# Black-Phoenix/CUDA-SfM

Hardware: AMD Instinct MI355X
Metric: RANSAC E-matrix hypotheses/sec (8-point, fused scoring), inlier-mask parity vs CPU oracle (higher is better)
Workload: dtype f32

## Files before the change

### cuda-sfm_amd/csrc/common.hpp

```cpp
#pragma once
#include <hip/hip_runtime.h>
#include <stdint.h>
#include <stddef.h>
#include <string>
#include <atomic>
#include <type_traits>
#include "../../include/sfm_amd.h"
#include "pair_state.hpp"
#include "job_order.hpp"
#if SFM_AB
#include "../../include/sfm_amd_ab.h"
#endif

#if SFM_AB
#define SFM_SW(p, i) ((p).reserved[i])
#else
#define SFM_SW(p, i) 0
#endif

namespace sfm {

void set_error(const char *fmt, ...);

#define SFM_HIP_TRY(expr)                                                                      \
// ... 143 lines not shown
    size_t views_floats = 0;
    hipEvent_t views_ev = nullptr;
    float pool_K[9] = {}, pool_Kinv[9] = {};
    float *pool_records = nullptr;
    size_t pool_records_cap = 0;
    void *batch_ws = nullptr;
    size_t batch_ws_bytes = 0;
    sfm::JobArray refine_jobs, register_jobs, view_points_jobs, adjust_jobs, align_jobs, fuse_jobs, chain_jobs, ring_jobs;
    void *fuse_ws = nullptr;
    size_t fuse_ws_bytes = 0;
    void *chain_ws = nullptr;
    size_t chain_ws_bytes = 0;
    void *ring_ws = nullptr;
    size_t ring_ws_bytes = 0;
    void *sift_job = nullptr;
    static constexpr int kBigLdsSlots = 16;
    const void *big_lds_done[kBigLdsSlots] = {};
};

inline int allow_big_lds(sfm_ctx *ctx, const void *kernel)
{
    for (int i = 0; i < sfm_ctx::kBigLdsSlots; ++i) {
        if (ctx->big_lds_done[i] == kernel) return SFM_OK;
        if (ctx->big_lds_done[i] == nullptr) {
            SFM_HIP_TRY(hipFuncSetAttribute(kernel, hipFuncAttributeMaxDynamicSharedMemorySize, 160 * 1024));
            ctx->big_lds_done[i] = kernel;
            return SFM_OK;
        }
    }
    SFM_HIP_TRY(hipFuncSetAttribute(kernel, hipFuncAttributeMaxDynamicSharedMemorySize, 160 * 1024));
    return SFM_OK;
}

struct ShardSlot {
    int *counts = nullptr;
    uint32_t *tick = nullptr;
    float *Ecand = nullptr;
    void *pf = nullptr;
    unsigned long long *key = nullptr;
    size_t cap_hyps = 0;
};

inline void shard_slot_free(ShardSlot &s)
{
    for (void *b : { (void *)s.counts, (void *)s.tick, (void *)s.Ecand, s.pf, (void *)s.key }) if (b) (void)hipFree(b);
    s = ShardSlot();
}

struct sfm_pair {
    sfm_ctx *ctx = nullptr;
    int image_count = 2;
    int n = 0;
    int cap_points = 0;
    int ld = 0;
    float *d_K = nullptr, *d_Kinv = nullptr;
    float *d_U[2] = { nullptr, nullptr };
    float *d_X[2] = { nullptr, nullptr };
    float4 *d_pts4 = nullptr;
    uint32_t sorted_epoch = 0;
    uint32_t pf_seen_epoch = 0;
    int pf_rule = 0;
    uint32_t *d_buckets = nullptr;
    size_t bucket_words = 0;
    uint32_t *d_tile_boxes = nullptr;
    int boxes_words = 0, boxes_tile = 0;
    float4 *d_pts4s = nullptr;
// ... 32 lines not shown
    float *d_vstate = nullptr;
    float *d_vreproj = nullptr;
    void *d_vwork = nullptr;
    void *d_vhyp = nullptr;
    int *d_vcounts = nullptr;
    size_t cap_vhyps = 0;
    uint32_t view_hyps = 0;
    void *d_awork = nullptr;
    void *d_lwork = nullptr;
    void *d_lhyp = nullptr;
    size_t cap_lhyps = 0;
    int last_kernel = 0, last_grid = 0, last_block = 0, last_lds = 0;
};

namespace sfm {

int match_db_rows(const sfm_ctx *ctx, int n2);
int match_records(sfm_ctx *ctx, sfm_sift_point *d_sift1, int n1, const sfm_sift_point *d_sift2, int n2, int *out_idx);
int pose_chain(sfm_pair *pair, int mode, float *d_record);

int lane_contexts(sfm_ctx *ctx, int n, sfm_ctx **out);
int start_lanes_after(sfm_ctx *ctx, sfm_ctx *const *lanes, int n, hipEvent_t event);

int launch_ransac_score(sfm_pair *pair, ShardSlot &slot, hipStream_t stream, const sfm_ransac_params &p, uint32_t h0, uint32_t count,
                        unsigned long long *key2 = nullptr, const float *d_E_given = nullptr, bool serial = true);
int launch_ransac_finalize(sfm_pair *pair, const sfm_ransac_params &p, const unsigned long long *d_key, uint32_t hyp_host, bool from_key,
                           hipStream_t stream = nullptr, bool rederive = false);
int launch_permutation_indices(sfm_ctx *ctx, int n, uint32_t seed, int32_t *d_indices);
bool prefilter_usable(const sfm_pair *pair, const sfm_ransac_params &p, uint32_t count);
int prefilter_pick_rule(sfm_pair *pair, const sfm_ransac_params &p, uint32_t count);
int launch_score_prefilter(sfm_pair *pair, ShardSlot &slot, hipStream_t stream, const sfm_ransac_params &p, uint32_t h0, uint32_t count, unsigned long long *key2);
bool prefilter_sums_counts(const sfm_pair *pair, const sfm_ransac_params &p, uint32_t count);
int launch_pf_prep(sfm_pair *pair, ShardSlot &slot, hipStream_t stream, const sfm_ransac_params &p, uint32_t count);
int prefilter_tile_points(const sfm_pair *pair, const sfm_ransac_params &p);
int launch_pf_cells(sfm_pair *pair, hipStream_t stream, bool want_sorted = false, int tile = 0);
#if SFM_AB
int launch_score_prefilter_r2(sfm_pair *pair, ShardSlot &slot, hipStream_t stream, const sfm_ransac_params &p, uint32_t h0, uint32_t count, unsigned long long *key2);
int launch_score_mfma(sfm_pair *pair, ShardSlot &slot, hipStream_t stream, const sfm_ransac_params &p, uint32_t h0, uint32_t count);
int launch_prefilter_probe(sfm_ctx *ctx, const float *d_E, float thr, float B, const float pt[4], int survive_all, float *d_out);
int launch_prefilter_band_probe(sfm_ctx *ctx, const float *d_E, float thr, float B, const float box[8], int b_safe, const float pt[4], int survive_all, float *d_out);
#endif
int launch_ransac_fused(sfm_pair *pair, ShardSlot &slot, hipStream_t stream, const sfm_ransac_params &p, uint32_t h0, uint32_t count);
int launch_finalize_block(sfm_pair *pair, const sfm_ransac_params &p, const unsigned long long *d_key, uint32_t hyp_host, bool from_key,
                          hipStream_t stream, bool rederive);

int launch_fill_xu(sfm_pair *pair, const sfm_sift_point *d_data);
int launch_set_points(sfm_pair *pair, const float *d_X0, const float *d_X1);
int launch_pose_candidates(sfm_pair *pair, int mode);
int launch_choose_pose(sfm_pair *pair, int mode);
int launch_triangulate(sfm_pair *pair, int mode);
int launch_points_to_vbo(sfm_pair *pair, float *d_positions, float *d_velocities, float scale);
int launch_pair_record(sfm_pair *pair, int mode, float *d_record);
int launch_pose_chain(sfm_pair *pair, float *d_record);

int launch_refine(sfm_pair *pair, const sfm_refine_params &p);
int launch_refine_pairs(sfm_ctx *ctx, sfm_pair *const *pairs, int num_pairs, const sfm_refine_params &p, const uint8_t *const *d_masks);
size_t refine_work_bytes(int cap_points);
int refine_state_words();
int refine_pose_offset();
int refine_report_offset();

int launch_register(sfm_pair *pair, const sfm_sift_point *d_sift, const sfm_register_params &p, const float *d_points, const uint8_t *d_valid);
int launch_register_views(sfm_ctx *ctx, sfm_pair *const *pairs, int num_pairs, const sfm_sift_point *const *d_sifts, const sfm_register_params &p,
                          const float *const *d_points, const uint8_t *const *d_valid);
size_t register_work_bytes(int cap_points);
size_t register_hyp_bytes(size_t num_hypotheses);
// ... 75 lines not shown
```

### cuda-sfm_amd/csrc/prefilter_lds.hpp

```cpp
#pragma once
#include "prefilter_record.hpp"

namespace sfm {

constexpr int kPfTileMax = 1024;
constexpr int kPfWaves = 16;
constexpr int kPfRing = 128;

constexpr int kPfERow = 10;
constexpr int kPfPassRows = 32, kPfPairRows = 64;
constexpr int pf_wave_bytes(int rows) { return rows * kPfERow * 4 + rows * 4; }
template <int RULE> struct PfLds {
    static constexpr int kFragsPerBlock = RULE == kPfRuleG ? 3 : 2;
    static constexpr int kBlockBytes = kFragsPerBlock * 64 * 16;
    static constexpr int kFrag = 0;
    static constexpr int kTileMax = kPfTileMax;
    int staged, pts, ring, wave, next, lut, bytes;
    __host__ __device__ explicit PfLds(int tile, int ring_entries = kPfRing, int entry_bytes = 8, int rows = RULE == kPfRuleG ? kPfPassRows : kPfPairRows)
    {
        staged = (tile + 63) & ~63;
        pts = kFrag + (staged / 32) * kBlockBytes;
        ring = pts + staged * 16;
        ring = (ring + ring_entries * entry_bytes - 1) & ~(ring_entries * entry_bytes - 1);
        wave = ring + kPfWaves * ring_entries * entry_bytes;
        next = wave + kPfWaves * pf_wave_bytes(rows);
        lut = next + 16;
        bytes = lut + kPfRingLutBytes;
    }
};
static_assert(kPfRing * 8 == 1024, "ring slots are addressed with (offset & 1023) | base");

static inline int pf_tile_points(int ld, int tmax)
{
    const int ntiles = (ld + tmax - 1) / tmax;
    const int t = ((ld + ntiles - 1) / ntiles + 31) & ~31;
    return t < 32 ? 32 : t;
}

constexpr unsigned long long kPfSumCountsMin = 1ull << 21;
static inline bool pf_sums_counts_at(unsigned count, int ld, int tile)
{
    return (unsigned long long)count * (unsigned long long)((ld + tile - 1) / tile) >= kPfSumCountsMin;
}

constexpr unsigned long long kPfPairPassesMin = 1ull << 22;
static inline bool pf_pairs_passes_at(unsigned count, int ld, int tile)
{
    return (unsigned long long)count * (unsigned long long)((ld + tile - 1) / tile) >= kPfPairPassesMin;
}

}
```

### cuda-sfm_amd/csrc/ransac.hip

```cpp
#include "ransac_device.hpp"
#include "block_ops.hpp"
#include "prefilter_record.hpp"

namespace sfm {

__device__ __forceinline__ void reset_keys(unsigned long long *key, unsigned long long *key2)
{
    if (blockIdx.x == 0 && threadIdx.x == 0) {
        key[0] = 0ull; key[1] = 0ull;
        if (key2) *key2 = 0ull;
    }
}

template <int WPE>
__global__ __launch_bounds__(64, WPE)
void ransac_solve_lanes(const float *__restrict__ X0, const float *__restrict__ X1, int ld, int n,
                        const int32_t *__restrict__ indices, uint32_t seed, uint32_t h0, uint32_t count,
                        int sweeps, float *__restrict__ Ecand, unsigned long long *zero_key, unsigned long long *zero_key2,
                        int *__restrict__ zero_counts, uint32_t *__restrict__ zero_ticks, uint32_t nzero)
{
    reset_keys(zero_key, zero_key2);
    const uint32_t i = blockIdx.x * blockDim.x + threadIdx.x;
    if (zero_ticks) for (uint32_t w = i; w < nzero; w += gridDim.x * blockDim.x) zero_ticks[w] = 0u;
    if (i >= count) return;
// ... 209 lines not shown
        unsigned long long b = sbest[0];
#pragma unroll
        for (int w = 1; w < WPB; ++w) b = sbest[w] > b ? sbest[w] : b;
        if (b) {
            atomicMax(best_key, b);
            if (best_key2) atomicMax(best_key2, b);
        }
    }
}

__global__ __launch_bounds__(256)
void ransac_argmax_counts(const int *__restrict__ counts, uint32_t h0, uint32_t count,
                          unsigned long long *best_key, unsigned long long *best_key2)
{
    __shared__ unsigned long long sbest[4];
    unsigned long long b = 0;
    for (uint32_t i = blockIdx.x * blockDim.x + threadIdx.x; i < count; i += gridDim.x * blockDim.x) {
        const unsigned long long key = pack_key((uint32_t)counts[i], h0 + i);
        b = key > b ? key : b;
    }
    b = wave_max(b);
    if ((threadIdx.x & 63) == 0) sbest[threadIdx.x >> 6] = b;
    __syncthreads();
    if (threadIdx.x == 0) {
#pragma unroll
        for (int w = 1; w < 4; ++w) b = sbest[w] > b ? sbest[w] : b;
        if (b) {
            atomicMax(best_key, b);
            if (best_key2) atomicMax(best_key2, b);
        }
    }
}

static size_t tick_words(size_t count) { return 2 * count + 64; }

static int ensure_hyp_capacity(ShardSlot &s, hipStream_t stream, size_t count)
{
    if (count <= s.cap_hyps) return SFM_OK;
    SFM_HIP_TRY(hipStreamSynchronize(stream));
    for (void *b : { (void *)s.counts, (void *)s.Ecand, (void *)s.tick, s.pf }) if (b) (void)hipFree(b);
    s.counts = nullptr; s.Ecand = nullptr; s.tick = nullptr; s.pf = nullptr; s.cap_hyps = 0;
    SFM_HIP_TRY(hipMalloc(&s.tick, tick_words(count) * sizeof(uint32_t)));
    SFM_HIP_TRY(hipMalloc(&s.pf, count * sizeof(PfRecord)));
    SFM_HIP_TRY(hipMalloc(&s.counts, count * sizeof(int)));
    SFM_HIP_TRY(hipMalloc(&s.Ecand, count * 9 * sizeof(float)));
    s.cap_hyps = count;
    return SFM_OK;
}

static int launch_argmax_counts(const ShardSlot &s, hipStream_t stream, uint32_t h0, uint32_t count, unsigned long long *key2)
{
    const int ablocks = (int)((count + 4095u) / 4096u);
    hipLaunchKernelGGL(ransac_argmax_counts, dim3(ablocks < 1024 ? ablocks : 1024), dim3(256), 0, stream, s.counts, h0, count, s.key, key2);
    SFM_HIP_TRY(hipGetLastError());
    return SFM_OK;
}

template <int WPB, bool UNITZ, int NH = 1, bool GRID2D = false>
static int launch_score_t(sfm_pair *pair, ShardSlot &s, hipStream_t stream, uint32_t h0, uint32_t count, float thr, int tile, int ntiles, int grid, size_t lds, unsigned long long *key2)
{
    const int rc_lds = allow_big_lds(pair->ctx, reinterpret_cast<const void *>(&ransac_score_waves<WPB, UNITZ, NH, GRID2D>));
    if (rc_lds != SFM_OK) return rc_lds;
    hipLaunchKernelGGL((ransac_score_waves<WPB, UNITZ, NH, GRID2D>), dim3(grid, GRID2D ? ntiles : 1), dim3(WPB * 64), lds, stream,
                       pair->d_X[0], pair->d_X[1], pair->ld, pair->n, s.Ecand, h0, count, thr, tile, ntiles,
                       s.counts, s.key, key2, pair->d_clk);
    SFM_HIP_TRY(hipGetLastError());
    if (GRID2D) {
        const int rca = launch_argmax_counts(s, stream, h0, count, key2);
// ... 31 lines not shown
    if (kernel == SFM_KERNEL_PREFILTER && !prefilter_usable(pair, p, 0x40000000u)) kernel = SFM_KERNEL_SPLIT;
    if (p.kernel == SFM_KERNEL_AUTO && kernel == SFM_KERNEL_SPLIT && prefilter_usable(pair, p, count) && SFM_SW(p, 3) != 1) kernel = SFM_KERNEL_PREFILTER;
    pair->last_kernel = kernel;
    if (kernel == SFM_KERNEL_FUSED) {
        rc = launch_ransac_fused(pair, s, stream, p, h0, count);
        if (rc == SFM_OK && key2) SFM_HIP_TRY(hipMemcpyAsync(key2, s.key, sizeof(unsigned long long), hipMemcpyDeviceToDevice, stream));
        return rc;
    }

    const int tile = pair->ld < kTileMax ? pair->ld : kTileMax;
    const int ntiles = (pair->ld + tile - 1) / tile;
    int wpb = 16;
    while (wpb > 4 && (count + wpb - 1) / wpb < (uint32_t)ctx->num_cus) wpb >>= 1;
    const int nh = (wpb == 16 && count >= 8192u) ? 2 : 1;
    const uint32_t nbatch = (count + wpb * nh - 1) / (wpb * nh);
    const bool grid2d = ntiles > 1 && kernel == SFM_KERNEL_SPLIT && wpb == 16 && SFM_SW(p, 1) != 1;
    const bool prefilter = kernel == SFM_KERNEL_PREFILTER;

    const bool timed = ctx->timing && ctx->tcount < sfm_ctx::kTimingSlots;
    hipEvent_t *tev = timed ? ctx->tev[ctx->tcount] : nullptr;
    if (timed) SFM_HIP_TRY(hipEventRecord(tev[0], stream));
    const bool pf_tickets = prefilter && (SFM_SW(p, 3) == 2 || SFM_SW(p, 3) == 17);
    const bool pf_r2 = prefilter && SFM_SW(p, 3) == 2;
    PfScales pf_sc = {};
    if (prefilter) (void)prefilter_scales(p.threshold, pf_sc);
    if (prefilter && !pf_r2) {
        const int pf_rule = prefilter_pick_rule(pair, p, count);
        const int rcc = launch_pf_cells(pair, stream, pf_rule == kPfRuleBandTile, prefilter_tile_points(pair, p));
        if (rcc != SFM_OK) return rcc;
    }
    const bool pf_sums = prefilter && !pf_r2 && !pf_tickets && prefilter_sums_counts(pair, p, count);
    int *zero_counts = (grid2d || pf_tickets || pf_sums) ? s.counts : nullptr;
    const float4 *pts4 = (pair->state.have_pts4 && SFM_SW(p, 0) != 4) ? pair->d_pts4 : nullptr;
    const uint32_t nzero = (!prefilter || pf_sums) ? 0u : (pf_tickets ? (count + (uint32_t)kPfGroup - 1u) / (uint32_t)kPfGroup : 2u * count);
    uint32_t *zero_ticks = (prefilter && !pf_sums) ? s.tick : nullptr;
    if (zero_ticks && d_E_given) {
        SFM_HIP_TRY(hipMemsetAsync(s.tick, 0, (size_t)nzero * sizeof(uint32_t), stream));
        zero_ticks = nullptr;
    }
    bool need_prep = prefilter && !pf_r2;
    if (d_E_given) {
        SFM_HIP_TRY(hipMemcpyAsync(s.Ecand, d_E_given, (size_t)count * 9 * sizeof(float), hipMemcpyDeviceToDevice, stream));
        if (zero_counts) SFM_HIP_TRY(hipMemsetAsync(s.counts, 0, (size_t)count * sizeof(int), stream));
    }
#if SFM_AB
    else if (p.reserved[0] == 1 || p.reserved[0] == 7) {
        auto kern = p.reserved[0] == 1 ? ransac_solve_lanes<1> : ransac_solve_lanes<3>;
        hipLaunchKernelGGL(kern, dim3((count + 63) / 64), dim3(64), 0, stream,
                           pair->d_X[0], pair->d_X[1], pair->ld, pair->n, p.d_indices, p.seed, h0, count,
                           p.jacobi_sweeps, s.Ecand, s.key, key2, zero_counts, zero_ticks, nzero);
    }
#endif
    else if (p.jacobi_sweeps <= 0 && (SFM_SW(p, 0) == 3 || (SFM_SW(p, 0) == 0 && (pts4 != nullptr || count <= kScalarSolveMax)))) {
        const bool fuse = need_prep && SFM_SW(p, 3) != 3;
        const bool tile_rec = !fuse || pair->pf_rule == kPfRuleBandTile;
        hipLaunchKernelGGL(tile_rec ? ransac_solve_lanes1_qr : ransac_solve_lanes1_qr_rec, dim3((count + 63) / 64), dim3(64), 0, stream,
                           pair->d_X[0], pair->d_X[1], pair->ld, pair->n, p.d_indices, p.seed, h0, count,
                           p.jacobi_sweeps, s.Ecand, s.key, key2, zero_counts, zero_ticks, nzero, pts4,
                           fuse ? reinterpret_cast<PfRecord *>(s.pf) : nullptr, p.threshold, pf_sc, pair->d_bound, pair->d_cells, pair->cells_mask,
                           pair->pf_rule);
        if (fuse) need_prep = false;
    }
    else if (p.jacobi_sweeps <= 0)
        hipLaunchKernelGGL(ransac_solve_lanes2<true>, dim3((count + 127) / 128), dim3(64), 0, stream,
                           pair->d_X[0], pair->d_X[1], pair->ld, pair->n, p.d_indices, p.seed, h0, count,
                           p.jacobi_sweeps, s.Ecand, s.key, key2, zero_counts, zero_ticks, nzero, pts4);
#if SFM_AB
    else if (p.reserved[0] == 2)
// ... 102 lines not shown
```

### cuda-sfm_amd/csrc/ransac_prefilter.hip

```cpp
#include "ransac_device.hpp"
#include "block_ops.hpp"
#include "prefilter_math.hpp"
#include "prefilter_record.hpp"
#include "prefilter_lds.hpp"

namespace sfm {

typedef float f16v __attribute__((ext_vector_type(16)));


__device__ constexpr int kPfESlot[9] = { 2, 6, 1, 3, 5, 7, 0, 4, 8 };
__device__ __forceinline__ uint32_t shift_in_reject(uint32_t rejected, float nt, float G)
{
    return __builtin_amdgcn_alignbit(rejected, __float_as_uint(fmaf(-nt, nt, G)), 31);
}

__device__ __forceinline__ uint32_t scan16(const f16v &nt, const f16v &G)
{
    uint32_t rejected = 0u;
#pragma unroll
    for (int r = 0; r < 16; ++r) rejected = shift_in_reject(rejected, nt[r], G[r]);
    return rejected;
}

// ... 113 lines not shown
                            const unsigned long long *__restrict__ bound_word, const uint32_t *__restrict__ tile_boxes)
{
    extern __shared__ __attribute__((aligned(16))) unsigned char smem[];
    const int lane = threadIdx.x & 63;
    const int wave = __builtin_amdgcn_readfirstlane(threadIdx.x >> 6);
    const bool probe = clk && blockIdx.x == 0 && blockIdx.y == 0 && threadIdx.x == 0;
    unsigned long long c0 = 0, w0 = 0;
    if (clk && blockIdx.x == 0 && blockIdx.y == 0 && wave == 0) { c0 = clock64(); w0 = wall_clock64(); }
#if SFM_AB
    const uint32_t trace_blk = blockIdx.y * gridDim.x + blockIdx.x;
    unsigned long long *trace = (clk && trace_blk < (uint32_t)kTraceBlocks) ? clk + 8 + (size_t)trace_blk * kTraceWords : nullptr;
    if (trace && threadIdx.x == 0) {
        trace[0] = wall_clock64();
        trace[2] = ((unsigned long long)__builtin_amdgcn_s_getreg((20 << 0) | (0 << 6) | (31 << 11)) << 32) |
                   (unsigned long long)__builtin_amdgcn_s_getreg((4 << 0) | (0 << 6) | (31 << 11));
        trace[3] = ((unsigned long long)blockIdx.y << 32) | blockIdx.x;
    }
#define PF_PHASE(k) do { if (probe1) clk[k] = wall_clock64() - w0; } while (0)
#else
#define PF_PHASE(k) do { } while (0)
#endif
    const int half = lane >> 5, row = lane & 31;
    uint32_t npass = (count + (uint32_t)kPfGroup - 1u) / (uint32_t)kPfGroup;
    const uint32_t nstatic = gridDim.x * (uint32_t)W;
    using LT = PfLds<RULE>;
    constexpr bool kBand = RULE != kPfRuleG, kTile = RULE == kPfRuleBandTile, kPack = RULE == kPfRuleBandPack || kTile;
    static_assert(!(FL2 && kPack) && !((VAR & kPfVarTickets) && kPack), "the recorded variants were built on the v_alignbit scan");
    constexpr bool kTail9 = kPack && W == 16 && !FL2 && !PIPE && !WIDE && !PRIO && !(VAR & kPfVarTickets);
    static_assert(kTail9 || (VAR & ~kPfVarTickets) == 0, "the pass-tail switches belong to the product's two rules");
    static_assert(!(VAR & kPfVarSinglePass) || (kTile && VAR == kPfVarSinglePass), "single passes: the per-tile rule's summing instance");
    static_assert(!(VAR & kPfVarPairDrain) || (kTile && VAR == kPfVarPairDrain), "paired passes drained between the scans: the per-tile rule's summing instance");
    constexpr bool kPair = kTile && kTail9 && (VAR == 0 || VAR == kPfVarPairDrain);
    constexpr bool kCarry = kPair && VAR == 0;
    constexpr int kRows = kPair ? kPfPairRows : kPfPassRows, kUnit = kRows;
    constexpr int kDrainMore = !kTail9 ? 0 : (VAR & kPfVarDrainK1) ? 1 : (VAR & kPfVarDrainK7) ? 7 : (VAR & kPfVarDrainLocal) ? 3 : 0;
    constexpr bool kDecodeTable = !(kTail9 && (VAR & kPfVarClosedDecode));
    constexpr bool kSumCounts = kTail9 && !(VAR & kPfVarAnswerEpilogue);
    constexpr int kRing = FL2 ? 256 : kPfRing;
    constexpr int kEnt = WIDE ? 16 : 8;
    static_assert(!WIDE || (kPack && !PIPE && !FL2), "wide entries: the packed scan's plain loop only");
    if (kPair) npass = (npass + 1u) >> 1;
    const LT L(tile, kRing, kEnt, kRows);
    float *etab = reinterpret_cast<float *>(smem + L.wave + wave * pf_wave_bytes(kRows));
    int *cnt = reinterpret_cast<int *>(etab + kRows * kPfERow);

    PfFrags afrag = {};
    h8 bfrag_n0 = {}, bfrag_n1 = {};
    uint32_t key0 = 0u;
    float rec_dn = 0.0f, rec_lin = 0.0f;
    float e_row[9] = {};
    auto fetch_pass = [&](uint32_t pass, PfFrags &af, uint32_t &k0, float (&e)[9], float &dn, float &lin) {
        const uint32_t hf = pass * (uint32_t)kUnit;
        const uint32_t h = hf + (uint32_t)min(kPair ? lane : row, (int)min((uint32_t)kUnit, count - hf) - 1);
        if (kTile) {
            const float *src = Ecand + 9 * (size_t)h;
#pragma unroll
            for (int k = 0; k < 9; ++k) e[k] = src[k];
            const uint4 rec = reinterpret_cast<const uint4 *>(recs)[h];
            k0 = rec.x; dn = __uint_as_float(rec.y); lin = __uint_as_float(rec.z);
            return;
        }
        const uint4 *r = reinterpret_cast<const uint4 *>(recs + h) + 2 * half;
        const uint4 r0 = r[0], r1 = r[1];
        if (kBand) pf_band_record_expand(r0, r1, half, af.n0, af.n1, k0);
        else pf_record_expand(r0, r1, half, af.n0, af.n1, af.t, k0);
        if (half == 0) {
// ... 86 lines not shown
            bfrag_n0 = __builtin_bit_cast(h8, ya); bfrag_n1 = __builtin_bit_cast(h8, yb);
        } else
        pf_tile_operands(e, fl, dn, lin, thr_l, B_l, tbox, half_l, afrag.n0, afrag.n1);
    };
    if (kTile) {
#pragma unroll
        for (int k = 0; k < 8; ++k) bw[k] = (uint32_t)__builtin_amdgcn_readlane((int)bw_lane, k);
        pf_B = uniform(pf_B);
        tbox = pf_box_from_bits(bw, pf_B);
        tbox = PfBox{ uniform(tbox.xlo), uniform(tbox.xhi), uniform(tbox.ylo), uniform(tbox.yhi), uniform(tbox.ulo), uniform(tbox.uhi), uniform(tbox.vlo), uniform(tbox.vhi) };
        if (have) build_operands(e_row, key0, rec_dn, rec_lin);
    }
#if SFM_AB
    if (probe) clk[2] = wall_clock64() - w0;
#endif
    const int npb = (min(tile, ld - tile_first) + 31) >> 5;
    const int npp = (npb + 1) >> 1;
    const float4 *pts = reinterpret_cast<const float4 *>(smem + L.pts);
    lds_cf *etab_l = (lds_cf *)etab;
    lds_i *cnt_l = (lds_i *)cnt;
    lds_cu8 *lut_l = (lds_cu8 *)(smem + L.lut);
    const uint32_t ring_base = (uint32_t)(size_t)(__attribute__((address_space(3))) unsigned char *)(smem + L.ring) + (uint32_t)wave * (uint32_t)(kRing * kEnt);
    uint32_t ring_mask = (uint32_t)(kRing * kEnt - 1);
    asm("" : "+v"(ring_mask));
    auto ring_at = [&](uint32_t index8) {
        return (lds_u2 *)((__attribute__((address_space(3))) unsigned char *)0 + ((index8 & ring_mask) | ring_base));
    };
    auto ring_at16 = [&](uint32_t index16) {
        return (lds_u4 *)((__attribute__((address_space(3))) unsigned char *)0 + ((index16 & ring_mask) | ring_base));
    };
    lds_ch8 *frag_lane = (lds_ch8 *)(smem + LT::kFrag) + lane;
    const ThrBand band = make_band(thr);
    uint32_t passes_done = 0;
#if SFM_AB
    uint32_t carried = 0;
#endif

    while (have) {
        SFM_PHASE("pass_begin");
        const uint32_t h_first = ps * (uint32_t)kUnit;
        const int nvalid_unit = (int)min((uint32_t)kUnit, count - h_first);
        int nvalid = min(nvalid_unit, kPfGroup), hoff = 0;
        const int nscan = (kPair && nvalid_unit > kPfGroup) ? 2 : 1;
#if SFM_AB
        const bool probe1 = probe && passes_done == 0u;
        unsigned long long w_scan_end = 0;
#endif
        uint32_t ps_next = ps + nstatic;
        if (dynamic) {
            uint32_t got = 0u;
            if (lane == 0) got = atomicAdd(next_idx, 1u);
            got = (uint32_t)__builtin_amdgcn_readfirstlane((int)got);
            ps_next = (got / (uint32_t)W) * nstatic + blockIdx.x * (uint32_t)W + (got % (uint32_t)W);
        }
        const unsigned long long scan_rows = __ballot(key0 != 0u);
        int head = 0, nq = 0;
        auto patch_zero_divisor_rows = [&](int sc) {
            uint32_t todo = kPair ? (uint32_t)(sc ? scan_rows >> 32 : scan_rows) : ((uint32_t)scan_rows | (uint32_t)(scan_rows >> 32));
            uint32_t survive = 0u;
            while (todo) {
                const int r = __builtin_ctz(todo) + hoff;
                todo &= todo - 1u;
                const float se[6] = { etab[6 * kRows + r], etab[2 * kRows + r], etab[r], etab[3 * kRows + r], etab[7 * kRows + r], etab[4 * kRows + r] };
                bool z = false;
                for (int j = 0; j < L.staged / 64; ++j) {
                    const float4 q = pts[j * 64 + lane];
                    z = z || prefilter_zero_divisor(se, q.x, q.z);
                }
                if (__ballot(z) != 0ull) survive |= 1u << (r - hoff);
            }
            if (survive != 0u && ((survive >> row) & 1u)) {
                const h8 zero = {};
                afrag.n0 = zero; afrag.n1 = zero; afrag.t = zero;
                if (half) { afrag.n1[3] = (_Float16)1.0f; afrag.t[7] = (_Float16)0.0009765625f; }
            }
        };

        uint32_t lane_tag = (uint32_t)(size_t)(lds_cf4 *)pts + (uint32_t)(row * 16) + (uint32_t)(half * 4);
        auto decide_first = [&](uint32_t &rest, uint32_t tag) {
            const int b = __builtin_clz(rest);
            rest &= ~(0x80000000u >> b);
            int hl, sub;
            if constexpr (kCarry) {
                const uint32_t code = (uint32_t)lut_l[pf_ring_lut_index(b, tag)];
                hl = (int)(code & 63u); sub = (int)(code >> 6);
            } else if (kPack) {
// ... 220 lines not shown
            mfma_step<RULE>(afrag, fa, g0, n0);
            const uint32_t rej_second = kBand ? scan16_band(n1) : scan16(n1, g1);
            PF_SCHED_STEP();
            __builtin_amdgcn_sched_barrier(0);
            const uint32_t rej32 = kBand ? (((rej_first << 1) & 0xAAAAAAAAu) | (rej_second & 0x55555555u))
                                                       : ((rej_first << 16) | rej_second);
            const bool mine = rej32 != 0xFFFFFFFFu;
            const unsigned long long any = __ballot(mine);
            SFM_PHASE("append_and_inloop_flush");
            if (any) {
                if (FL2) { while (nq >= 128) flush2(); }
                else
                while (nq >= 64) flush(64, kInLoop);
                const int slot = __builtin_amdgcn_mbcnt_hi((uint32_t)(any >> 32), __builtin_amdgcn_mbcnt_lo((uint32_t)any, 0u));
                if (mine) *ring_at(((uint32_t)(head + nq) + (uint32_t)slot) * 8u) = u2v{ ~rej32, lane_tag + ((uint32_t)pp << 10) };
                nq += __builtin_popcountll(any);
            }
        }
        }
        if (sc + 1 >= nscan) break;
#if SFM_AB
        if (probe1) w_scan_end = wall_clock64();
#endif
        if constexpr (kCarry) lane_tag |= kPfTagScan;
        else while (nq > 0) flush(min(nq, 64), kDrain);
#if SFM_AB
        carried += (uint32_t)nq;
#endif
        afrag.n0 = bfrag_n0; afrag.n1 = bfrag_n1;
        hoff = kPfGroup; nvalid = nvalid_unit - kPfGroup;
        }
        PF_PHASE(4);
        SFM_PHASE("pass_end_fetch_next");
        const bool have_next = ps_next < npass;
        PfFrags afrag_next = afrag;
        uint32_t key0n = 0u;
        float e_next[9] = {}, dn_next = 0.0f, lin_next = 0.0f;
        if (have_next) fetch_pass(ps_next, afrag_next, key0n, e_next, dn_next, lin_next);
        SFM_PHASE("drain_flush");
        if (FL2) { while (nq >= 128) flush2(); }
        if (WIDE) { while (nq > 0) flush_w(min(nq, 64)); }
        while (nq > 0) flush(min(nq, 64), kDrain);
        SFM_PHASE("epilogue");
        PF_PHASE(7);
        if (VAR & kPfVarTickets) {
        if (lane < nvalid) {
            const int c = cnt[lane];
            if (c) atomicAdd(&counts[h_first + lane], c);
        }
        asm volatile("s_waitcnt vmcnt(0)" ::: "memory");
        uint32_t t = 0;
        if (lane == 0) t = atomicAdd(&tick[ps], 1u);
        t = __builtin_amdgcn_readfirstlane(t);
        if (t == gridDim.y - 1) {
            unsigned long long k = 0;
            if (lane < nvalid) {
                const int c = __hip_atomic_load(&counts[h_first + lane], __ATOMIC_RELAXED, __HIP_MEMORY_SCOPE_AGENT);
                k = pack_key((uint32_t)c, h0 + h_first + (uint32_t)lane);
            }
            k = wave_max(k);
            if (lane == 0 && k) {
                atomicMax(best_key, k);
                if (best_key2) atomicMax(best_key2, k);
            }
        }
        } else if (kSumCounts) {
// ... 17 lines not shown
        const int nvalid_done = nvalid;
        const uint32_t h_done = h_first;
        if (have_next) {
            if (kTile) build_operands(e_next, key0n, dn_next, lin_next);
            else { afrag = afrag_next; key0 = key0n; }
            install_rows(e_next);
        }
        unsigned long long k = 0;
        if (lane < nvalid_done && (uint32_t)(old >> 32) == gridDim.y - 1u) {
            const uint32_t total = (uint32_t)old + c_mine;
            counts[h_done + lane] = (int)total;
            k = pack_key(total, h0 + h_done + (uint32_t)lane);
        }
        if (__ballot(k != 0ull) != 0ull) {
            k = wave_max(k);
            if (lane == 0 && k > __hip_atomic_load(best_key, __ATOMIC_RELAXED, __HIP_MEMORY_SCOPE_AGENT)) {
                atomicMax(best_key, k);
                if (best_key2) atomicMax(best_key2, k);
            }
        }
        }
        PF_PHASE(5);
        ++passes_done;
        have = have_next;
        if (have_next) {
            ps = ps_next;
            if (VAR & kPfVarTickets) { afrag = afrag_next; key0 = key0n; install_rows(e_next); }
        }
    }
    SFM_PHASE("kernel_end");
    if (probe) { clk[6] = passes_done; clk[0] = clock64() - c0; clk[1] = wall_clock64() - w0; }
#if SFM_AB
    if (probe) clk[6] |= (unsigned long long)carried << 32;
    if (trace && lane == 0) {
        const unsigned long long tend = wall_clock64();
        trace[4 + wave] = tend;
        if (wave == 0) trace[1] = tend;
    }
#endif
}

constexpr int kPfBuckets = 1024 + 2;
constexpr int kPfBucketBlock = 256;

__device__ __forceinline__ int pf_bucket_of(const float4 q, float B)
{
    const float big = fmaxf(fmaxf(fabsf(q.x), fabsf(q.y)), fmaxf(fabsf(q.z), fabsf(q.w)));
    if (!(big <= 48.0f) || q.x != q.x || q.y != q.y || q.z != q.z || q.w != q.w) return kPfBuckets - 2;
    return (int)(pf_morton_key(q.x, q.y, -B, B, -B, B) >> 20);
}

__global__ __launch_bounds__(1024)
void pf_bucket_scan_kernel(uint32_t *__restrict__ hist, int nblocks, uint32_t *__restrict__ base, uint32_t *__restrict__ boxes, int nbox_words)
{
    for (int k = threadIdx.x; k < nbox_words; k += blockDim.x) boxes[k] = pf_order_bits(-INFINITY);
    __shared__ uint32_t total[kPfBuckets + 1024];
    for (int b = threadIdx.x; b < kPfBuckets; b += blockDim.x) {
        uint32_t run = 0u;
        for (int k = 0; k < nblocks; ++k) {
            const uint32_t c = hist[(size_t)k * kPfBuckets + b];
            hist[(size_t)k * kPfBuckets + b] = run;
            run += c;
        }
        total[b] = run;
    }
    __syncthreads();
    __shared__ uint32_t wsum[17];
    base[threadIdx.x] = block_scan<16>(total[threadIdx.x], wsum);
    if (threadIdx.x == 0) { base[1024] = wsum[16]; base[1025] = wsum[16] + total[1024]; }
// ... 341 lines not shown
}

constexpr uint64_t kPfOrderFirstCallPairs = 1ull << 33;
int prefilter_pick_rule(sfm_pair *pair, const sfm_ransac_params &p, uint32_t count)
{
    int rule = pf_rule_switch(p);
    if (rule < 0) {
        const bool ordered = pair->sorted_epoch == pair->bound_epoch && pair->d_pts4s != nullptr;
        const bool first = pair->pf_seen_epoch != pair->bound_epoch;
        rule = (!ordered && first && (uint64_t)count * (uint64_t)pair->ld < kPfOrderFirstCallPairs) ? kPfRuleBandPack : kPfRuleBandTile;
    }
    pair->pf_seen_epoch = pair->bound_epoch;
    pair->pf_rule = rule;
    return rule;
}

bool prefilter_usable(const sfm_pair *pair, const sfm_ransac_params &p, uint32_t count)
{
    PfScales sc;
    return pair->state.unit_z && pair->state.have_bound && count >= 16384u && (uint64_t)count * (uint64_t)pair->ld >= (1ull << 27) && prefilter_scales(p.threshold, sc);
}

static int pf_tile_of(const sfm_pair *pair, const sfm_ransac_params &p)
{
    if (SFM_SW(p, 1) == 7 && pair->pf_rule == kPfRuleBand) return pf_tile_points(pair->ld, 1536);
    return pf_tile_points(pair->ld, kPfTileMax);
}

int prefilter_tile_points(const sfm_pair *pair, const sfm_ransac_params &p) { return pf_tile_of(pair, p); }

static int pf_tail_var(const sfm_pair *pair, const sfm_ransac_params &p, uint32_t count)
{
    const bool large = pf_sums_counts_at(count, pair->ld, pf_tile_of(pair, p));
    if (SFM_SW(p, 1) == 19) return 0;
    if (SFM_SW(p, 1) == 20) return pair->pf_rule == kPfRuleBandTile ? kPfVarSinglePass : 0;
    if (SFM_SW(p, 1) == 21) return pair->pf_rule == kPfRuleBandTile ? kPfVarPairDrain : 0;
    if (pair->pf_rule == kPfRuleBandTile && SFM_SW(p, 1) == 16) return kPfVarDrainK1;
    if (pair->pf_rule == kPfRuleBandTile && SFM_SW(p, 1) == 17) return kPfVarDrainK7;
    int var = 0;
    const bool lab = SFM_SW(p, 3) >= 8 && SFM_SW(p, 3) < 16;
    if (lab && (SFM_SW(p, 3) & 1)) var |= kPfVarDrainLocal;
    if (lab && (SFM_SW(p, 3) & 2)) var |= kPfVarClosedDecode;
    const bool sum = (lab && (SFM_SW(p, 3) & 4)) ? false : (large || (SFM_SW(p, 1) >= 16 && SFM_SW(p, 1) <= 18));
    if (!sum) var |= kPfVarAnswerEpilogue;
    if (var == 0 && pair->pf_rule == kPfRuleBandTile && !pf_pairs_passes_at(count, pair->ld, pf_tile_of(pair, p))) var = kPfVarSinglePass;
    return var;
}

bool prefilter_sums_counts(const sfm_pair *pair, const sfm_ransac_params &p, uint32_t count)
{
    const bool product_rule = pair->pf_rule == kPfRuleBandTile || pair->pf_rule == kPfRuleBandPack;
    const bool variant = SFM_SW(p, 1) == 5 || (SFM_SW(p, 1) >= 11 && SFM_SW(p, 1) <= 15);
    return product_rule && !variant && !(pf_tail_var(pair, p, count) & kPfVarAnswerEpilogue);
}

int launch_score_prefilter(sfm_pair *pair, ShardSlot &s, hipStream_t stream, const sfm_ransac_params &p, uint32_t h0, uint32_t count, unsigned long long *key2)
{
    sfm_ctx *ctx = pair->ctx;
    PfScales sc;
    if (!prefilter_scales(p.threshold, sc)) { set_error("threshold %g outside the pre-filter's range", (double)p.threshold); return SFM_E_INVALID; }
    const int waves = (SFM_SW(p, 1) == 5 || SFM_SW(p, 1) == 12) ? 12 : kPfWaves;
    const int tile = pf_tile_of(pair, p);
    const int ntiles = (pair->ld + tile - 1) / tile;
    const uint32_t npass = (count + (uint32_t)kPfGroup - 1u) / (uint32_t)kPfGroup;
    const int rule = pair->pf_rule;
    const int tail_var = pf_tail_var(pair, p, count);
    const bool wide = rule == kPfRuleBandTile && SFM_SW(p, 1) == 13;
    const bool paired_units = rule == kPfRuleBandTile && (tail_var == 0 || tail_var == kPfVarPairDrain) && waves == kPfWaves && !wide && SFM_SW(p, 1) != 14 && SFM_SW(p, 1) != 15;
    const uint32_t nunits = paired_units ? (npass + 1u) / 2u : npass;
    const uint32_t iters = (nunits + (uint32_t)waves - 1) / (uint32_t)waves;
    uint32_t cols = (uint32_t)ctx->num_cus / (uint32_t)ntiles;
    if (SFM_SW(p, 2) > 0) cols = (uint32_t)SFM_SW(p, 2);
    if (cols > iters) cols = iters;
    if (cols < 1) cols = 1;
    const int dynamic = SFM_SW(p, 1) == 2 ? 0 : 1;
    const int var = SFM_SW(p, 3) >= 16 ? SFM_SW(p, 3) - 16 : 0;
    const bool fl2 = rule == kPfRuleBand && waves == kPfWaves && SFM_SW(p, 1) == 9;
    const int lds_bytes = wide ? PfLds<kPfRuleBand>(tile, kPfRing, 16, kPfPassRows).bytes : fl2 ? PfLds<kPfRuleBand>(tile, 256, 8, kPfPassRows).bytes
                        : rule != kPfRuleG ? PfLds<kPfRuleBand>(tile, kPfRing, 8, paired_units ? kPfPairRows : kPfPassRows).bytes : PfLds<kPfRuleG>(tile).bytes;
    if (lds_bytes > 160 * 1024) { set_error("pre-filter tile of %d points needs %d bytes of LDS", tile, lds_bytes); return SFM_E_INVALID; }
    auto launch = [&](auto kernel) -> int {
        const int rc_lds = allow_big_lds(ctx, reinterpret_cast<const void *>(kernel));
        if (rc_lds != SFM_OK) return rc_lds;
        const float *x0 = rule == kPfRuleBandTile ? reinterpret_cast<const float *>(pair->d_pts4s) : pair->d_X[0];
        hipLaunchKernelGGL(kernel, dim3(cols, ntiles), dim3(waves * 64), lds_bytes, stream,
                           x0, pair->d_X[1], pair->ld, pair->n, s.Ecand, reinterpret_cast<const PfRecord *>(s.pf), h0, count, p.threshold,
                           dynamic, tile, s.counts, s.tick, s.key, key2, pair->d_clk, pair->d_bound, pair->d_tile_boxes);
        return SFM_OK;
    };
    int rcl;
#if SFM_AB
    if (rule == kPfRuleG && waves == 12) rcl = launch(&ransac_score_prefilter<12, 0, kPfRuleG>);
    else if (rule == kPfRuleG && var == 1) rcl = launch(&ransac_score_prefilter<16, 1, kPfRuleG>);
    else if (rule == kPfRuleG) rcl = launch(&ransac_score_prefilter<16, 0, kPfRuleG>);
    else if (waves == 12) rcl = launch(&ransac_score_prefilter<12, 0, kPfRuleBand>);
    else if (fl2) rcl = launch(&ransac_score_prefilter<16, 0, kPfRuleBand, 1>);
    else if (rule == kPfRuleBand) rcl = launch(&ransac_score_prefilter<16, 0, kPfRuleBand>);
    else if (SFM_SW(p, 1) == 11) rcl = launch(&ransac_score_prefilter<16, 0, kPfRuleBandPack, 0, 1>);
    else if (SFM_SW(p, 1) == 12) rcl = launch(&ransac_score_prefilter<12, 0, kPfRuleBandPack, 0, 1>);
    else if (wide) rcl = launch(&ransac_score_prefilter<16, 0, kPfRuleBandTile, 0, 0, 1>);
    else if (rule == kPfRuleBandTile && SFM_SW(p, 1) == 14) rcl = launch(&ransac_score_prefilter<16, 0, kPfRuleBandTile, 0, 0, 0, 1>);
    else if (rule == kPfRuleBandTile && SFM_SW(p, 1) == 15) rcl = launch(&ransac_score_prefilter<16, 0, kPfRuleBandTile, 0, 0, 0, 2>);
    else if (tail_var != 0 && tail_var != kPfVarAnswerEpilogue && tail_var != kPfVarSinglePass) {
        rcl = SFM_E_INVALID;
#define PF_TAIL_CASE(V) case V: rcl = rule == kPfRuleBandPack ? launch(&ransac_score_prefilter<16, V, kPfRuleBandPack>) : launch(&ransac_score_prefilter<16, V, kPfRuleBandTile>); break
        switch (tail_var) {
        PF_TAIL_CASE(2); PF_TAIL_CASE(4); PF_TAIL_CASE(6); PF_TAIL_CASE(10); PF_TAIL_CASE(12); PF_TAIL_CASE(14);
        case kPfVarDrainK1: rcl = launch(&ransac_score_prefilter<16, kPfVarDrainK1, kPfRuleBandTile>); break;
// ... 22 lines not shown
```

### profiles/trace_probe.py

```python
import json, os, sys
import numpy as np
sys.path.insert(0, os.path.dirname(os.path.dirname(os.path.abspath(__file__))))
import torch
import cuda_sfm_amd_ab as S
from cuda_sfm_amd_ab import synth

dev = torch.device("cuda", 0)
ctx = S.Context(0, torch.cuda.current_stream().cuda_stream)
SW1 = [int(a[6:]) for a in sys.argv[1:] if a.startswith("--sw1=")]
sys.argv = [a for a in sys.argv if not a.startswith("--sw1=")]
cases = [(4096, int(h)) for h in sys.argv[1:]] or [(4096, 1 << 20), (4096, 131072), (16384, 1 << 20)]
for n, H in cases:
    scene = synth.two_view_scene(n)
    d_sift = torch.from_numpy(scene["sift"].view(np.uint8).reshape(n, 576)).to(dev)
    pair = S.ImagePair(ctx, scene["K"], scene["Kinv"], 2, n)
    pair.fillXU(d_sift)
    p = S.default_params(n, num_hypotheses=H, kernel=S.KERNEL_PREFILTER)
    if SW1:
        p.reserved[1] = SW1[0]
    for _ in range(10):
        pair.ransac_score(p)
    torch.cuda.synchronize()
    t = pair.last_trace().astype(np.float64)
    us = 0.01
    start, wave_end = t[:, 0] * us, t[:, 4:20] * us
    t0 = start.min()
    start -= t0; wave_end -= t0
    blk_end = wave_end.max(axis=1)
    life = blk_end - start
    span = blk_end.max()
    xcc = (t[:, 2].astype(np.uint64) >> np.uint64(32)).astype(int) & 0xF
    spread = wave_end.max(axis=1) - wave_end.min(axis=1)
    live = (wave_end - start[:, None]).sum() / (span * len(t))
    out = {"sw1": SW1[0] if SW1 else 0, "matches": n, "hypotheses": H, "blocks": len(t), "span_us": round(span, 1), "last_start_us": round(float(start.max()), 1),
           "block_lifetime_us_p0_10_50_90_100": [round(float(x), 1) for x in np.percentile(life, [0, 10, 50, 90, 100])],
           "block_end_us_p10_50_90": [round(float(x), 1) for x in np.percentile(blk_end, [10, 50, 90])],
           "wave_end_spread_in_block_us_p50_90_100": [round(float(x), 1) for x in np.percentile(spread, [50, 90, 100])],
           "mean_live_waves_per_block_over_span": round(float(live), 2),
           "lifetime_by_xcc_us": {int(x): round(float(life[xcc == x].mean()), 1) for x in sorted(set(xcc))},
           "blocks_by_xcc": {int(x): int((xcc == x).sum()) for x in sorted(set(xcc))}}
    print(json.dumps(out), flush=True)
    pair.close()
```

Baseline: 2.907 billion.

## Add per-tile shared work queue for tail rounds of prefilter scoring

Splits the prefilter's dynamic work handout into two parts. Waves first take units by position from the per-column ticket for the first three quarters of the rounds. After that, they draw from a per-tile global atomic queue shared across all columns, so blocks that finish early can take work from slower columns and the tail becomes more even. This adds a second atomic per queued pass, plus zeroing of the queue words in the tick buffer. It only applies to the paired-unit band-tile summing instance, and debug switches select alternative handout rules.

```diff
diff --git a/cuda-sfm_amd/csrc/common.hpp b/cuda-sfm_amd/csrc/common.hpp
--- a/cuda-sfm_amd/csrc/common.hpp
+++ b/cuda-sfm_amd/csrc/common.hpp
@@ -199,6 +199,7 @@
     return SFM_OK;
 }
 
+inline size_t tick_words(size_t count) { return 2 * count + 64; }
 struct ShardSlot {
     int *counts = nullptr;
     uint32_t *tick = nullptr;
@@ -297,6 +298,7 @@
 int launch_score_prefilter(sfm_pair *pair, ShardSlot &slot, hipStream_t stream, const sfm_ransac_params &p, uint32_t h0, uint32_t count, unsigned long long *key2);
 bool prefilter_sums_counts(const sfm_pair *pair, const sfm_ransac_params &p, uint32_t count);
 int launch_pf_prep(sfm_pair *pair, ShardSlot &slot, hipStream_t stream, const sfm_ransac_params &p, uint32_t count);
+uint32_t prefilter_queue_words(const sfm_pair *pair, const sfm_ransac_params &p, uint32_t count);
 int prefilter_tile_points(const sfm_pair *pair, const sfm_ransac_params &p);
 int launch_pf_cells(sfm_pair *pair, hipStream_t stream, bool want_sorted = false, int tile = 0);
 #if SFM_AB
diff --git a/cuda-sfm_amd/csrc/prefilter_lds.hpp b/cuda-sfm_amd/csrc/prefilter_lds.hpp
--- a/cuda-sfm_amd/csrc/prefilter_lds.hpp
+++ b/cuda-sfm_amd/csrc/prefilter_lds.hpp
@@ -49,4 +49,33 @@
     return (unsigned long long)count * (unsigned long long)((ld + tile - 1) / tile) >= kPfPairPassesMin;
 }
 
+#define PF_UNIT_BY_POSITION(ticket, w, nstatic, col) (((ticket) / (uint32_t)(w)) * (nstatic) + (col) * (uint32_t)(w) + ((ticket) % (uint32_t)(w)))
+constexpr unsigned kPfQueueRoundsMin = 4;
+constexpr int kPfQueueLineWords = 32;
+enum { kPfHandoutProduct = 0, kPfHandoutStatic = 1, kPfHandoutFirstRound = 2, kPfHandoutHalf = 3, kPfHandoutThreeQuarters = 4 };
+struct PfHandout {
+    unsigned rounds, rounds_static, nstatic, w;
+    SFM_HD PfHandout(unsigned nunits, unsigned cols, unsigned waves, int rule = kPfHandoutProduct)
+    {
+        w = waves;
+        nstatic = cols * waves;
+        rounds = (nunits + nstatic - 1u) / nstatic;
+        unsigned rs = rounds;
+        if (rule == kPfHandoutProduct) rs = rounds < kPfQueueRoundsMin ? rounds : 3u * rounds / 4u;
+        else if (rule == kPfHandoutThreeQuarters) rs = 3u * rounds / 4u;
+        else if (rule == kPfHandoutHalf) rs = rounds / 2u;
+        else if (rule == kPfHandoutFirstRound) rs = 1u;
+        rounds_static = rs < 1u ? 1u : rs > rounds ? rounds : rs;
+    }
+    SFM_HD bool queued() const { return rounds_static < rounds; }
+    SFM_HD unsigned first_queue_ticket() const { return rounds_static * w; }
+    SFM_HD unsigned kernel_ticket() const { return queued() ? first_queue_ticket() : 0x7FFFFFFFu; }
+    SFM_HD static uint32_t unit_by_position(uint32_t nstatic, uint32_t w, uint32_t col, uint32_t ticket) { return PF_UNIT_BY_POSITION(ticket, w, nstatic, col); }
+    SFM_HD static unsigned unit_from_queue(unsigned first_queue_ticket, unsigned cols, unsigned g) { return first_queue_ticket * cols + g; }
+    SFM_HD unsigned unit(unsigned col, unsigned ticket, unsigned g) const
+    {
+        return ticket < kernel_ticket() ? unit_by_position(nstatic, w, col, ticket) : unit_from_queue(first_queue_ticket(), nstatic / w, g);
+    }
+};
+
 }
diff --git a/cuda-sfm_amd/csrc/ransac.hip b/cuda-sfm_amd/csrc/ransac.hip
--- a/cuda-sfm_amd/csrc/ransac.hip
+++ b/cuda-sfm_amd/csrc/ransac.hip
@@ -265,8 +265,6 @@
     }
 }
 
-static size_t tick_words(size_t count) { return 2 * count + 64; }
-
 static int ensure_hyp_capacity(ShardSlot &s, hipStream_t stream, size_t count)
 {
     if (count <= s.cap_hyps) return SFM_OK;
@@ -364,8 +362,9 @@
     const bool pf_sums = prefilter && !pf_r2 && !pf_tickets && prefilter_sums_counts(pair, p, count);
     int *zero_counts = (grid2d || pf_tickets || pf_sums) ? s.counts : nullptr;
     const float4 *pts4 = (pair->state.have_pts4 && SFM_SW(p, 0) != 4) ? pair->d_pts4 : nullptr;
-    const uint32_t nzero = (!prefilter || pf_sums) ? 0u : (pf_tickets ? (count + (uint32_t)kPfGroup - 1u) / (uint32_t)kPfGroup : 2u * count);
-    uint32_t *zero_ticks = (prefilter && !pf_sums) ? s.tick : nullptr;
+    const uint32_t pf_queue = pf_sums ? prefilter_queue_words(pair, p, count) : 0u;
+    const uint32_t nzero = !prefilter ? 0u : pf_sums ? pf_queue : (pf_tickets ? (count + (uint32_t)kPfGroup - 1u) / (uint32_t)kPfGroup : 2u * count);
+    uint32_t *zero_ticks = (prefilter && nzero) ? s.tick : nullptr;
     if (zero_ticks && d_E_given) {
         SFM_HIP_TRY(hipMemsetAsync(s.tick, 0, (size_t)nzero * sizeof(uint32_t), stream));
         zero_ticks = nullptr;
diff --git a/cuda-sfm_amd/csrc/ransac_prefilter.hip b/cuda-sfm_amd/csrc/ransac_prefilter.hip
--- a/cuda-sfm_amd/csrc/ransac_prefilter.hip
+++ b/cuda-sfm_amd/csrc/ransac_prefilter.hip
@@ -169,6 +169,7 @@
     static_assert(!(VAR & kPfVarPairDrain) || (kTile && VAR == kPfVarPairDrain), "paired passes drained between the scans: the per-tile rule's summing instance");
     constexpr bool kPair = kTile && kTail9 && (VAR == 0 || VAR == kPfVarPairDrain);
     constexpr bool kCarry = kPair && VAR == 0;
+    constexpr bool kQueue = kCarry;
     constexpr int kRows = kPair ? kPfPairRows : kPfPassRows, kUnit = kRows;
     constexpr int kDrainMore = !kTail9 ? 0 : (VAR & kPfVarDrainK1) ? 1 : (VAR & kPfVarDrainK7) ? 7 : (VAR & kPfVarDrainLocal) ? 3 : 0;
     constexpr bool kDecodeTable = !(kTail9 && (VAR & kPfVarClosedDecode));
@@ -321,8 +322,10 @@
     lds_ch8 *frag_lane = (lds_ch8 *)(smem + LT::kFrag) + lane;
     const ThrBand band = make_band(thr);
     uint32_t passes_done = 0;
+    [[maybe_unused]] uint32_t drawn = 0u;
 #if SFM_AB
     uint32_t carried = 0;
+    uint32_t queue_draws = 0;
 #endif
 
     while (have) {
@@ -336,11 +339,20 @@
         unsigned long long w_scan_end = 0;
 #endif
         uint32_t ps_next = ps + nstatic;
+        [[maybe_unused]] uint32_t queued = 0u;
         if (dynamic) {
             uint32_t got = 0u;
             if (lane == 0) got = atomicAdd(next_idx, 1u);
             got = (uint32_t)__builtin_amdgcn_readfirstlane((int)got);
-            ps_next = (got / (uint32_t)W) * nstatic + blockIdx.x * (uint32_t)W + (got % (uint32_t)W);
+            ps_next = PF_UNIT_BY_POSITION(got, W, nstatic, blockIdx.x);
+            if constexpr (kQueue) {
+                queued = (uint32_t)__builtin_amdgcn_readfirstlane(got >= (uint32_t)dynamic ? 1 : 0);
+                if (queued && lane == 0) {
+                    uint32_t word = (uint32_t)kPfQueueLineWords * blockIdx.y;
+                    asm volatile("" : "+v"(word));
+                    drawn = __hip_atomic_fetch_add(tick + word, 1u, __ATOMIC_RELAXED, __HIP_MEMORY_SCOPE_AGENT);
+                }
+            }
         }
         const unsigned long long scan_rows = __ballot(key0 != 0u);
         int head = 0, nq = 0;
@@ -627,6 +639,14 @@
         }
         PF_PHASE(4);
         SFM_PHASE("pass_end_fetch_next");
+        if constexpr (kQueue) {
+            if (queued) {
+                ps_next = PfHandout::unit_from_queue((uint32_t)dynamic, gridDim.x, (uint32_t)__builtin_amdgcn_readfirstlane((int)drawn));
+#if SFM_AB
+                queue_draws += 1u + (ps_next < npass ? 0x10000u : 0u);
+#endif
+            }
+        }
         const bool have_next = ps_next < npass;
         PfFrags afrag_next = afrag;
         uint32_t key0n = 0u;
@@ -710,9 +730,10 @@
     if (probe) { clk[6] = passes_done; clk[0] = clock64() - c0; clk[1] = wall_clock64() - w0; }
 #if SFM_AB
     if (probe) clk[6] |= (unsigned long long)carried << 32;
+    if (probe) clk[5] = (clk[5] & 0xFFFFFFFFull) | ((unsigned long long)queue_draws << 32);
     if (trace && lane == 0) {
         const unsigned long long tend = wall_clock64();
-        trace[4 + wave] = tend;
+        trace[4 + wave] = (tend & 0x00FFFFFFFFFFFFFFull) | ((unsigned long long)min(passes_done, 255u) << 56);
         if (wave == 0) trace[1] = tend;
     }
 #endif
@@ -1120,7 +1141,7 @@
 static int pf_tail_var(const sfm_pair *pair, const sfm_ransac_params &p, uint32_t count)
 {
     const bool large = pf_sums_counts_at(count, pair->ld, pf_tile_of(pair, p));
-    if (SFM_SW(p, 1) == 19) return 0;
+    if (SFM_SW(p, 1) == 19 || (SFM_SW(p, 1) >= 22 && SFM_SW(p, 1) <= 25)) return 0;
     if (SFM_SW(p, 1) == 20) return pair->pf_rule == kPfRuleBandTile ? kPfVarSinglePass : 0;
     if (SFM_SW(p, 1) == 21) return pair->pf_rule == kPfRuleBandTile ? kPfVarPairDrain : 0;
     if (pair->pf_rule == kPfRuleBandTile && SFM_SW(p, 1) == 16) return kPfVarDrainK1;
@@ -1142,26 +1163,53 @@
     return product_rule && !variant && !(pf_tail_var(pair, p, count) & kPfVarAnswerEpilogue);
 }
 
+static int pf_handout_rule(const sfm_ransac_params &p)
+{
+    return SFM_SW(p, 1) >= 22 && SFM_SW(p, 1) <= 25 ? SFM_SW(p, 1) - 22 + kPfHandoutStatic : kPfHandoutProduct;
+}
+static bool pf_queue_instance(int rule, int tail_var, bool paired_units) { return rule == kPfRuleBandTile && tail_var == 0 && paired_units; }
+struct PfLaunchShape { int waves, tile, ntiles, tail_var; bool paired_units; uint32_t npass, nunits, cols; };
+static PfLaunchShape pf_grid_of(const sfm_pair *pair, const sfm_ransac_params &p, uint32_t count)
+{
+    PfLaunchShape g;
+    g.waves = (SFM_SW(p, 1) == 5 || SFM_SW(p, 1) == 12) ? 12 : kPfWaves;
+    g.tile = pf_tile_of(pair, p);
+    g.ntiles = (pair->ld + g.tile - 1) / g.tile;
+    g.npass = (count + (uint32_t)kPfGroup - 1u) / (uint32_t)kPfGroup;
+    g.tail_var = pf_tail_var(pair, p, count);
+    const bool wide = pair->pf_rule == kPfRuleBandTile && SFM_SW(p, 1) == 13;
+    g.paired_units = pair->pf_rule == kPfRuleBandTile && (g.tail_var == 0 || g.tail_var == kPfVarPairDrain) && g.waves == kPfWaves && !wide && SFM_SW(p, 1) != 14 && SFM_SW(p, 1) != 15;
+    g.nunits = g.paired_units ? (g.npass + 1u) / 2u : g.npass;
+    const uint32_t iters = (g.nunits + (uint32_t)g.waves - 1) / (uint32_t)g.waves;
+    g.cols = (uint32_t)pair->ctx->num_cus / (uint32_t)g.ntiles;
+    if (SFM_SW(p, 2) > 0) g.cols = (uint32_t)SFM_SW(p, 2);
+    if (g.cols > iters) g.cols = iters;
+    if (g.cols < 1) g.cols = 1;
+    return g;
+}
+
+uint32_t prefilter_queue_words(const sfm_pair *pair, const sfm_ransac_params &p, uint32_t count)
+{
+    const PfLaunchShape g = pf_grid_of(pair, p, count);
+    if (!pf_queue_instance(pair->pf_rule, g.tail_var, g.paired_units) || SFM_SW(p, 1) == 2) return 0u;
+    const uint32_t words = (uint32_t)kPfQueueLineWords * (uint32_t)g.ntiles;
+    if ((size_t)words > tick_words(count)) return 0u;
+    return PfHandout(g.nunits, g.cols, (unsigned)g.waves, pf_handout_rule(p)).queued() ? words : 0u;
+}
+
 int launch_score_prefilter(sfm_pair *pair, ShardSlot &s, hipStream_t stream, const sfm_ransac_params &p, uint32_t h0, uint32_t count, unsigned long long *key2)
 {
     sfm_ctx *ctx = pair->ctx;
     PfScales sc;
     if (!prefilter_scales(p.threshold, sc)) { set_error("threshold %g outside the pre-filter's range", (double)p.threshold); return SFM_E_INVALID; }
-    const int waves = (SFM_SW(p, 1) == 5 || SFM_SW(p, 1) == 12) ? 12 : kPfWaves;
-    const int tile = pf_tile_of(pair, p);
-    const int ntiles = (pair->ld + tile - 1) / tile;
-    const uint32_t npass = (count + (uint32_t)kPfGroup - 1u) / (uint32_t)kPfGroup;
-    const int rule = pair->pf_rule;
-    const int tail_var = pf_tail_var(pair, p, count);
+    const PfLaunchShape g = pf_grid_of(pair, p, count);
+    const int waves = g.waves, tile = g.tile, ntiles = g.ntiles, rule = pair->pf_rule, tail_var = g.tail_var;
     const bool wide = rule == kPfRuleBandTile && SFM_SW(p, 1) == 13;
-    const bool paired_units = rule == kPfRuleBandTile && (tail_var == 0 || tail_var == kPfVarPairDrain) && waves == kPfWaves && !wide && SFM_SW(p, 1) != 14 && SFM_SW(p, 1) != 15;
-    const uint32_t nunits = paired_units ? (npass + 1u) / 2u : npass;
-    const uint32_t iters = (nunits + (uint32_t)waves - 1) / (uint32_t)waves;
-    uint32_t cols = (uint32_t)ctx->num_cus / (uint32_t)ntiles;
-    if (SFM_SW(p, 2) > 0) cols = (uint32_t)SFM_SW(p, 2);
-    if (cols > iters) cols = iters;
-    if (cols < 1) cols = 1;
-    const int dynamic = SFM_SW(p, 1) == 2 ? 0 : 1;
+    const bool paired_units = g.paired_units;
+    const uint32_t nunits = g.nunits, cols = g.cols;
+    int dynamic = SFM_SW(p, 1) == 2 ? 0 : 1;
+    if (dynamic && pf_queue_instance(rule, tail_var, paired_units))
+        dynamic = (int)PfHandout(nunits, cols, (unsigned)waves, prefilter_queue_words(pair, p, count) ? pf_handout_rule(p) : kPfHandoutStatic).kernel_ticket();
     const int var = SFM_SW(p, 3) >= 16 ? SFM_SW(p, 3) - 16 : 0;
     const bool fl2 = rule == kPfRuleBand && waves == kPfWaves && SFM_SW(p, 1) == 9;
     const int lds_bytes = wide ? PfLds<kPfRuleBand>(tile, kPfRing, 16, kPfPassRows).bytes : fl2 ? PfLds<kPfRuleBand>(tile, 256, 8, kPfPassRows).bytes
diff --git a/profiles/handout_ab.py b/profiles/handout_ab.py
--- /dev/null
+++ b/profiles/handout_ab.py
@@ -0,0 +1,53 @@
+import json
+import os
+import subprocess
+import sys
+import time
+
+ROOT = os.path.dirname(os.path.dirname(os.path.abspath(__file__)))
+
+if sys.argv[1] == "run":
+    sys.path.insert(0, ROOT)
+    import numpy as np
+    import torch
+    import cuda_sfm_amd_ab as S
+    from cuda_sfm_amd_ab import synth
+    n, H, sw = int(sys.argv[2]), int(sys.argv[3]), int(sys.argv[4])
+    dev = torch.device("cuda", 0)
+    scene = synth.two_view_scene(n)
+    d_sift = torch.from_numpy(scene["sift"].view(np.uint8).reshape(n, 576)).to(dev)
+    ctx = S.Context(0, torch.cuda.current_stream().cuda_stream)
+    ctx.own_stream()
+    pair = S.ImagePair(ctx, scene["K"], scene["Kinv"], 2, n)
+    pair.fillXU(d_sift)
+    p = S.default_params(n, num_hypotheses=H, kernel=S.KERNEL_PREFILTER)
+    p.reserved[1] = sw
+    for _ in range(20):
+        pair.estimateE_pipelined(p)
+    pair.flush(); ctx.synchronize(); torch.cuda.synchronize()
+    steps = 200 if n <= 4096 else 60
+    t0 = time.perf_counter()
+    for _ in range(steps):
+        pair.estimateE_pipelined(p)
+    pair.flush(); ctx.synchronize(); torch.cuda.synchronize()
+    dt = (time.perf_counter() - t0) / steps
+    launch = pair.last_launch()
+    draws = int(pair.last_phases()[5]) >> 32
+    print(json.dumps({"matches": n, "hypotheses": H, "reserved1": sw, "ms_per_step": dt * 1e3, "grid": launch["grid"], "best": list(pair.get_best()),
+                      "queue_draws_wave0_block0": draws & 0xFFFF, "queue_units_wave0_block0": draws >> 16}))
+    sys.exit(0)
+
+n, H, switches = int(sys.argv[1]), int(sys.argv[2]), [int(s) for s in sys.argv[3].split(",")]
+reps = int(sys.argv[4]) if len(sys.argv) > 4 else 3
+out = open(sys.argv[5], "w") if len(sys.argv) > 5 else None
+for rep in range(reps):
+    for sw in switches:
+        r = subprocess.run(["timeout", "-k", "10", "120", sys.executable, os.path.abspath(__file__), "run", str(n), str(H), str(sw)], cwd=ROOT, capture_output=True, text=True)
+        lines = [ln for ln in r.stdout.splitlines() if ln.startswith("{")]
+        if r.returncode != 0 or not lines:
+            print("FAILED", sw, r.returncode, r.stdout[-1500:], r.stderr[-3000:], flush=True)
+            sys.exit(1)
+        msg = json.dumps({"rep": rep, **json.loads(lines[-1])})
+        print(msg, flush=True)
+        if out:
+            out.write(msg + "\n"); out.flush()
diff --git a/profiles/trace_probe.py b/profiles/trace_probe.py
--- a/profiles/trace_probe.py
+++ b/profiles/trace_probe.py
@@ -21,7 +21,12 @@
     for _ in range(10):
         pair.ransac_score(p)
     torch.cuda.synchronize()
-    t = pair.last_trace().astype(np.float64)
+    raw = pair.last_trace().astype(np.uint64)
+    units = (raw[:, 4:20] >> np.uint64(56)).astype(int).sum(axis=1)
+    raw[:, 4:20] &= np.uint64((1 << 56) - 1)
+    t = raw.astype(np.float64)
+    tile_of = (raw[:, 3] >> np.uint64(32)).astype(int)
+    draws = int(pair.last_phases()[5]) >> 32
     us = 0.01
     start, wave_end = t[:, 0] * us, t[:, 4:20] * us
     t0 = start.min()
@@ -38,6 +43,11 @@
            "wave_end_spread_in_block_us_p50_90_100": [round(float(x), 1) for x in np.percentile(spread, [50, 90, 100])],
            "mean_live_waves_per_block_over_span": round(float(live), 2),
            "lifetime_by_xcc_us": {int(x): round(float(life[xcc == x].mean()), 1) for x in sorted(set(xcc))},
-           "blocks_by_xcc": {int(x): int((xcc == x).sum()) for x in sorted(set(xcc))}}
+           "blocks_by_xcc": {int(x): int((xcc == x).sum()) for x in sorted(set(xcc))},
+           "lifetime_by_tile_us": {int(x): round(float(life[tile_of == x].mean()), 1) for x in sorted(set(tile_of))},
+           "end_by_tile_us_mean_max": {int(x): [round(float(blk_end[tile_of == x].mean()), 1), round(float(blk_end[tile_of == x].max()), 1)] for x in sorted(set(tile_of))},
+           "units_per_block_p0_10_50_90_100": [int(x) for x in np.percentile(units, [0, 10, 50, 90, 100])],
+           "units_per_block_by_xcc": {int(x): round(float(units[xcc == x].mean()), 1) for x in sorted(set(xcc))},
+           "queue_draws_wave0_block0": draws & 0xFFFF, "queue_units_wave0_block0": draws >> 16}
     print(json.dumps(out), flush=True)
     pair.close()
```

New measurement: 2.912 billion, median of 6. About the same (+0.2%).
